# batmanlab/Mammo-CLIP

Measured on AMD Instinct MI355X. Metric: image-text pairs/s (whole node), EN-B5+BioClinicalBERT contrastive pre-training step, higher is better.
Workload: dtype bf16; 1 GPU; cfg4: efficientnet-b5 + BioClinicalBERT(BERT-base), 1024 pairs/GPU (2 views + 2 reports each), 1520x912 images, 256-token reports, breast_clip loss, AdamW; fwd+loss+bwd+optimizer; dropout/drop-connect on; global_batch=1024, parallelism=dp1 x 32 micro-batches, keep_graphs=7, recompute=0, keep_recompute=2, stat_tapes=True, streams=3

## Files before the change

### include/mammoclip_hip.h

```cpp
#ifndef MAMMOCLIP_HIP_H
#define MAMMOCLIP_HIP_H
#include <stdint.h>
#ifdef __cplusplus
extern "C" {
#endif

typedef uint16_t mc_bf16;

const char* mc_last_error(void);
int mc_version(void);
int mc_storage_is_f16(void);

typedef struct mc_gemm_args {
    const mc_bf16* A;
    const mc_bf16* B;
    void* C;
    long long M, K;
    int N;
    long long lda, ldb, ldc;
    int a_kmajor, b_kmajor;
    int c_f32, c_atomic;
    int splits;
    int batch, nb2;
    long long sA1, sA2, sB1, sB2, sC1, sC2;
// ... 28 lines not shown
int mc_quant_fp8_bf16(const mc_bf16* x, long long n, const float* amax_in, unsigned char* y, float* scale_out,
                      float* amax_next, void* stream);

typedef struct mc_gemm_rows_args {
    const mc_bf16* X;
    long long M;
    int K;
    long long ldx;
    const mc_bf16* W;
    int N;
    long long ldw;
    mc_bf16* C;
    long long ldc;
    const mc_bf16* R;
    long long ldr;
    const float* pro_scale;
    const float* pro_shift;
    const float* pro_gate;
    long long pro_rows_per_img;
    float* stat_partials;
    const float* bias;
    int epi_mode;
    const mc_bf16* epi_x;
    long long epi_ldx;
    long long epi_rows_per_img;
    const float* epi_scale;
    const float* epi_shift;
    const float* epi_mean;
    const float* epi_invstd;
    const float* epi_coef;
    const float* epi_mul;
    const float* epi_add;
    float epi_add_scale;
    float* epi_sums;
    float* epi_ws;
} mc_gemm_rows_args;
int mc_gemm_rows_supported(int n, int k);
long long mc_gemm_rows_epi_ws_floats(const mc_gemm_rows_args* args);
int mc_gemm_rows_epi_supported(long long M, int N, int K, long long rows_per_img, int epi_mode);
int mc_gemm_rows_blocks(const mc_gemm_rows_args* args);
int mc_gemm_rows_bf16(const mc_gemm_rows_args* args, void* stream);

typedef struct mc_wgrad_rows_args {
    const mc_bf16* dY;
    int N;
    long long lddy;
    const mc_bf16* X;
    int K;
    long long ldx;
    long long M;
    float* dW;
    float* ws;
    int accumulate;
    const float* pro_scale;
    const float* pro_shift;
    const float* pro_gate;
    long long pro_rows_per_img;
} mc_wgrad_rows_args;
int mc_wgrad_rows_supported(int n, int k);
int mc_wgrad_rows_blocks(long long m);
int mc_wgrad_rows_bf16(const mc_wgrad_rows_args* args, void* stream);
int mc_xbwd_rows_supported(int n, int k);
int mc_xbwd_rows_blocks(long long m);
int mc_xbwd_rows_bf16(const mc_wgrad_rows_args* args, const mc_bf16* wt, long long ldwt, mc_bf16* dx, long long lddx,
                      const mc_bf16* r, long long ldr, void* stream);

int mc_cast_f32_bf16(const float* src, mc_bf16* dst, long long n, void* stream);
int mc_cast_f32_bf16_lo(const float* src, mc_bf16* dst, long long n, void* stream);
int mc_cast_bf16_f32(const mc_bf16* src, float* dst, long long n, void* stream);
int mc_transpose_f32(const float* src, float* dst, int rows, int cols, void* stream);
int mc_cast_transpose_f32_bf16(const float* src, mc_bf16* dst, int rows, int cols, void* stream);
int mc_stem_weight_prep(const float* w, mc_bf16* out, int c0, void* stream);

int mc_stem_im2col(const float* x, long long sn, long long sc, long long sh, long long sw,
                   int n, int h, int w, int pad_l, int pad_t, int oh, int ow, mc_bf16* out, void* stream);
int mc_gate_weights_bf16(const mc_bf16* w, const float* gate, int n_img, int n, int k, mc_bf16* out, void* stream);

int mc_image_minmax_u8(const unsigned char* x, long long sn, long long elems_per_image, int n,
                       unsigned int* minmax, void* stream);
int mc_stem_im2col_u8(const unsigned char* x, long long sn, long long sc, long long sh, long long sw,
                      const unsigned int* minmax, float mean, float std, int n, int h, int w, int pad_l,
                      int pad_t, int oh, int ow, mc_bf16* out, void* stream);

typedef struct mc_dwconv_args {
    const mc_bf16* x;
    const mc_bf16* dy;
    void* out;
    const float* w_kkc;
    int n, h, w, c;
    int k, stride, pad_l, pad_t, oh, ow;
    const float* pro_scale;
    const float* pro_shift;
    float* stat_partials;
    const mc_bf16* epi_x;
    const float* epi_scale;
    const float* epi_shift;
    const float* epi_mean;
    const float* epi_invstd;
    float* dw_out;
    int stat_rows;
    const mc_bf16* xw;
    int cin;
} mc_dwconv_args;
int mc_dwconv_stat_rows(const mc_dwconv_args* args);
int mc_dwconv_bwd_data_stat_rows(const mc_dwconv_args* args);
int mc_dwconv_fwd(const mc_dwconv_args* args, void* stream);
int mc_dwconv_bwd_data(const mc_dwconv_args* args, void* stream);
int mc_dwconv_bwd_weight(const mc_dwconv_args* args, void* stream);
int mc_dwconv_bwd_data_xw_supported(const mc_dwconv_args* args);
int mc_dwconv_bwd_data_plan(const mc_dwconv_args* args, int* plan);
int mc_dwconv_bwd_data_xw_preferred(const mc_dwconv_args* args);
int mc_dwconv_set_lane_mode(int mode);
int mc_dwconv_lane_supported(const mc_dwconv_args* args);
int mc_dwconv_bwd_fused_supported(const mc_dwconv_args* args);
int mc_dwconv_bwd_fused_preferred(const mc_dwconv_args* args);
int mc_dwconv_bwd_fused_stat_rows(const mc_dwconv_args* args);
int mc_dwconv_bwd_fused(const mc_dwconv_args* args, void* stream);
int mc_mbconv_xdw_supported(const mc_dwconv_args* args);
int mc_mbconv_xdw_stat_rows(const mc_dwconv_args* args);
int mc_mbconv_xdw_fwd(const mc_dwconv_args* args, void* stream);

int mc_bn_finalize(const float* partials, int rows, int c, double count, const float* gamma,
                   const float* beta, float* running_mean, float* running_var, float momentum, float eps,
                   int update_running, float* mean, float* invstd, float* scale, float* shift, void* stream);
int mc_bn_eval_coeffs(const float* gamma, const float* beta, const float* running_mean,
                      const float* running_var, float eps, int c, float* scale, float* shift, void* stream);

typedef struct mc_bnact_args {
    const mc_bf16* x;
    long long n_img, hw;
    int c;
    const float* scale;
    const float* shift;
    int act;
    const float* rowscale;
    const mc_bf16* res;
    mc_bf16* out;
    float* pooled;
    const mc_bf16* g;
    const float* mul;
    const float* add;
    float add_scale;
    const float* mean;
    const float* invstd;
    float* partials;
    const float* coef;
    mc_bf16* dx;
    float* dgate;
    float* split_ws;
} mc_bnact_args;
int mc_bnact_rows(const mc_bnact_args* args);
int mc_bnact_img_splits(const mc_bnact_args* args);
int mc_bnact_apply(const mc_bnact_args* args, void* stream);
int mc_bnact_pool(const mc_bnact_args* args, void* stream);
int mc_bnact_bwd_reduce(const mc_bnact_args* args, void* stream);
int mc_bnact_bwd_apply(const mc_bnact_args* args, void* stream);
int mc_bnact_se_dgate(const mc_bnact_args* args, void* stream);
int mc_bnact_se_sums(const mc_bnact_args* args, void* stream);
int mc_bn_partials_from_se_sums(const float* sums, const float* gate, const float* dpooled, float add_scale,
                                long long n_img, int c, float* partials, void* stream);
int mc_bn_bwd_finalize(const float* partials, int rows, int c, double count, const float* gamma,
                       const float* mean, const float* invstd, float* dgamma, float* dbeta, float* coef,
                       void* stream);

int mc_bn_fold_prepare(const float* we, const float* coef, const float* xtx, const float* colsum_x, double rows, int n,
                       int k, mc_bf16* w1t, mc_bf16* wb, mc_bf16* sxx, void* stream);
// ... 135 lines not shown
```

### mammo_clip_amd/breastclip/model/modules/efficientnet_custom.py

```python
import math
from collections import namedtuple
from typing import List, Optional

import os

import torch
from torch import nn

from .... import ops

BN_MOMENTUM = 0.01
BN_EPS = 1e-3

VALID_MODELS = tuple(f"efficientnet-b{i}" for i in range(9)) + ("efficientnet-l2",)

_COEFFS = {
    "efficientnet-b0": (1.0, 1.0, 224, 0.2), "efficientnet-b1": (1.0, 1.1, 240, 0.2),
    "efficientnet-b2": (1.1, 1.2, 260, 0.3), "efficientnet-b3": (1.2, 1.4, 300, 0.3),
    "efficientnet-b4": (1.4, 1.8, 380, 0.4), "efficientnet-b5": (1.6, 2.2, 456, 0.4),
    "efficientnet-b6": (1.8, 2.6, 528, 0.5), "efficientnet-b7": (2.0, 3.1, 600, 0.5),
    "efficientnet-b8": (2.2, 3.6, 672, 0.5), "efficientnet-l2": (4.3, 5.3, 800, 0.5),
}
_STAGES = ((1, 3, 1, 1, 32, 16), (2, 3, 2, 6, 16, 24), (2, 5, 2, 6, 24, 40), (3, 3, 2, 6, 40, 80),
           (3, 5, 1, 6, 80, 112), (4, 5, 2, 6, 112, 192), (1, 3, 1, 6, 192, 320))
# ... 73 lines not shown
    _TAPE = tape


def _replaying():
    return _TAPE is not None and _TAPE.mode == "replay"


class _BNDefer:

    def __init__(self, enc):
        offs, tot = {}, 0
        for bn in enc._bn_layers:
            offs[id(bn)] = tot
            tot += bn.num_features
        self.offs, self.total = offs, tot
        self.flat = torch.zeros(2 * tot, dtype=torch.float32, device=enc._ones_b.device)
        self.used = []

    def scratch(self, bn):
        o, c = self.offs[id(bn)], bn.num_features
        self.used.append(bn)
        return self.flat[o:o + c], self.flat[self.total + o:self.total + o + c]

    @torch.no_grad()
    def apply(self):
        if not self.used:
            return
        if self.flat.is_cuda:
            self.flat.record_stream(torch.cuda.current_stream(self.flat.device))
        dst = [bn.running_mean for bn in self.used] + [bn.running_var for bn in self.used]
        src = [self.flat[self.offs[id(bn)]:self.offs[id(bn)] + bn.num_features] for bn in self.used] + \
              [self.flat[self.total + self.offs[id(bn)]:self.total + self.offs[id(bn)] + bn.num_features] for bn in self.used]
        torch._foreach_mul_(dst, 1.0 - BN_MOMENTUM)
        torch._foreach_add_(dst, src)
        self.used = []


_BN_DEFER = None


def _bn_stats(partials, count, bn: nn.BatchNorm2d, training: bool):
    if training:
        if _replaying():
            return _TAPE.get()
        if _BN_DEFER is not None and bn.track_update:
            rm, rv = _BN_DEFER.scratch(bn)
        else:
            rm, rv = bn.running_mean, bn.running_var
        st = ops.bn_finalize(partials, count, bn.weight, bn.bias, rm, rv, BN_MOMENTUM, BN_EPS, bn.track_update)
        if bn.track_update:
            if bn.defer_count is not None:
                bn.defer_count.append(bn.num_batches_tracked)
            else:
                bn.num_batches_tracked += 1
        if _TAPE is not None:
            _TAPE.put(st)
        return st
    return ops.bn_eval_coeffs(bn.weight, bn.bias, bn.running_mean, bn.running_var, BN_EPS)


def _conv_stats(fn, training, *a, stats=True, **kw):
    if not stats or (training and _replaying()):
        return fn(*a, **kw), None
    return fn(*a, stats=True, **kw)


LINK_STEM = os.environ.get("MC_LINK_STEM", "1") != "0"
FUSE_DW_BWD = os.environ.get("MC_FUSE_DW_BWD", "1") != "0"
FUSE_PROJ_DGRAD = os.environ.get("MC_FUSE_PROJ_DGRAD", "1") != "0"
BN_FOLD_MIN_BYTES = int(os.environ.get("MC_BN_FOLD_MIN_BYTES", 250_000_000))
BN_FOLD_S2_MIN_BYTES = int(os.environ.get("MC_BN_FOLD_S2_MIN_BYTES", 0))
XDW_MAX_CIN = int(os.environ.get("MC_XDW_MAX_CIN", 64))
MODE3_MAX_CEXP = int(os.environ.get("MC_MODE3_MAX_CEXP", 1 << 30))


class _StemFn(torch.autograd.Function):

    @staticmethod
    def forward(ctx, x, w, gamma, beta, mod, link=None):
        n, _, h, wd = x.shape
        l, r, t, b = mod.stem_pad
        _, oh, ow = mod.stem_geo(n, h, wd)
        c0 = w.shape[0]
        patches = ops.stem_im2col(x, l, t, oh, ow)
        wb = ops.stem_weight_prep(w)
        training = mod.training
        e, part = _conv_stats(ops.linear_fwd, training, patches, wb)
        st = _bn_stats(part, n * oh * ow, mod._bn0, training)
        ctx.mod, ctx.st, ctx.geo = mod, st, (n, h, wd, oh, ow, c0)
        ctx.raw = (x.mean, x.std) if isinstance(x, ops.RawImages) else None
        ctx.save_for_backward(x.data if ctx.raw else x, e)
        ctx.link = link
        if link is not None:
            link.st, link.part = st, None
            return e.detach()
        return ops.bnact_apply(e, n, oh * ow, c0, st.scale, st.shift, 1)

    @staticmethod
    def backward(ctx, dy):
        x, e = ctx.saved_tensors
        if ctx.raw:
            x = ops.RawImages(x, *ctx.raw)
        n, h, wd, oh, ow, c0 = ctx.geo
        mod = ctx.mod
        link = ctx.link
        if link is not None:
            de, dgamma, dbeta = ops.bnact_bwd(e, n, oh * ow, c0, ctx.st, mod._bn0.weight, 0, g=dy.contiguous(), partials=link.part)
            link.part = None
        else:
            de, dgamma, dbeta = ops.bnact_bwd(e, n, oh * ow, c0, ctx.st, mod._bn0.weight, 1, g=dy.contiguous())
        l, r, t, b = mod.stem_pad
        patches = ops.stem_im2col(x, l, t, oh, ow)
        dw = ops.linear_wgrad(de, patches)
        gw, gg, gb = ops.deliver_param_grads((mod._conv_stem.weight, mod._bn0.weight, mod._bn0.bias),
                                             (dw[:, :27].reshape(c0, 3, 3, 3), dgamma, dbeta))
        return (None, gw, gg, gb, None) + ((None,) if link is not None else ())


class _StemLink:
    __slots__ = ("st", "part")

    def __init__(self):
        self.st, self.part = None, None


def _expand_conv(pl, x, we, stats=True):
    if pl.fp8_expand:
        return ops.linear_fwd_fp8(x, we, stats=True)
    return _conv_stats(ops.linear_fwd, pl.training, x, we, stats=stats)


def _depthwise(blk, pl, x, e, we, wkkc, pro0, stats=True):
    if pl.xdw:
        return _conv_stats(ops.mbconv_xdw_fwd, pl.training, x, we, pro0, wkkc, *pl.dw, stats=stats)
    return _conv_stats(ops.dwconv_fwd, pl.training, e if blk.args.expand != 1 else x, wkkc, *pl.dw, stats=stats, pro=pro0)


def _project_conv(pl, d, act1, st1, gate, wp, stats=True):
    ohw = pl.oh * pl.ow
    if pl.fp8_project:
        wg = ops.gate_weights(wp, gate)
        return ops.linear_fwd_fp8(act1, wg, stats=True, batch_w=(pl.n, ohw))
    src, pro = (act1, (None, None, gate, ohw)) if pl.keep_act else (d, (st1.scale, st1.shift, gate, ohw))
    return _conv_stats(ops.linear_fwd, pl.training, src, wp, stats=stats, pro=pro)


class _MBConvFn(torch.autograd.Function):

    @staticmethod
    def forward(ctx, x, rowscale, blk, n, h, w, recording, link, *params):
        a = blk.args
        pl = blk.plan(n, h, w, recording)
        training, ohw = pl.training, pl.oh * pl.ow
        wkkc = blk.w_taps()
        e = we = st0 = gram = None
        if a.expand != 1:
            we = blk.w_expand()
            if pl.xdw:
                if training and _replaying():
                    part0, gram = None, _TAPE.get()
                elif training:
                    part0, gram = ops.bn_gram_partials(x, we, n * h * w)
                    if _TAPE is not None:
                        _TAPE.put(gram)
                else:
                    part0 = None
            else:
                e, part0 = _expand_conv(pl, x, we)
            st0 = _bn_stats(part0, n * h * w, blk._bn0, training)
            pro0 = (st0.scale, st0.shift)
        else:
            pro0 = (link.st.scale, link.st.shift) if link is not None else None
        d, part1 = _depthwise(blk, pl, x, e, we, wkkc, pro0)
        st1 = _bn_stats(part1, n * ohw, blk._bn1, training)
        if pl.keep_act:
            pooled, act1 = ops.bnact_pool(d, n, ohw, a.cexp, st1.scale, st1.shift, 1, keep_act=True)
        elif training and _replaying():
            pooled, act1 = _TAPE.get(), None
        else:
            pooled, act1 = ops.bnact_pool(d, n, ohw, a.cexp, st1.scale, st1.shift, 1), None
            if training and _TAPE is not None:
                _TAPE.put(pooled)
        if training and _replaying():
            gate = _TAPE.get()
        else:
            gate = ops.se_fwd(pooled, blk._se_reduce.weight.view(a.cse, a.cexp), blk._se_reduce.bias,
                              blk._se_expand.weight.view(a.cexp, a.cse), blk._se_expand.bias)
            if training and _TAPE is not None:
                _TAPE.put(gate)
        wp = blk.w_project()
        p, part2 = _project_conv(pl, d, act1, st1, gate, wp)
        st2 = _bn_stats(part2, n * ohw, blk._bn2, training)
        y = ops.bnact_apply(p, n, ohw, a.cout, st2.scale, st2.shift, 0,
                            rowscale=rowscale if a.skip else None, res=x if a.skip else None)
        ctx.blk, ctx.plan, ctx.saved = blk, pl, dict(
            x=x, e=e if pl.store_e else None, d=d if pl.store_d else None, act1=act1 if pl.store_d else None,
# ... 522 lines not shown
```

### mammo_clip_amd/lib.py

```python
import ctypes as C
import os

_HERE = os.path.dirname(os.path.abspath(__file__))
STORAGE = os.environ.get("MC_STORAGE", "bf16").lower()
if STORAGE not in ("bf16", "f16"):
    raise ValueError(f"MC_STORAGE must be 'bf16' or 'f16', got {STORAGE!r}")
LIB_PATH = os.path.join(_HERE, "lib", "libmammoclip_hip.so" if STORAGE == "bf16" else "libmammoclip_hip_f16.so")

P, LL, I, F, D, U, ULL = C.c_void_p, C.c_longlong, C.c_int, C.c_float, C.c_double, C.c_uint, C.c_ulonglong


class GemmArgs(C.Structure):
    _fields_ = [
        ("A", P), ("B", P), ("C", P),
        ("M", LL), ("K", LL), ("N", I),
        ("lda", LL), ("ldb", LL), ("ldc", LL),
        ("a_kmajor", I), ("b_kmajor", I),
        ("c_f32", I), ("c_atomic", I),
        ("splits", I),
        ("batch", I), ("nb2", I),
        ("sA1", LL), ("sA2", LL), ("sB1", LL), ("sB2", LL), ("sC1", LL), ("sC2", LL),
        ("bias", P), ("bias_stride1", LL),
        ("act", I),
        ("R", P), ("ldr", LL),
        ("alpha", F),
        ("pro_operand", I),
        ("pro_scale", P), ("pro_shift", P), ("pro_gate", P),
        ("pro_rows_per_img", LL), ("pro_nch", I),
        ("stat_partials", P),
        ("max_grid_m", I),
        ("splitk_ws", P),
        ("split_group_rows", LL), ("split_sub", I), ("split_scale", P),
        ("ab_fp8", I), ("alpha_dev", P),
    ]


class GemmRowsArgs(C.Structure):
    _fields_ = [
        ("X", P), ("M", LL), ("K", I), ("ldx", LL),
        ("W", P), ("N", I), ("ldw", LL),
        ("C", P), ("ldc", LL),
        ("R", P), ("ldr", LL),
        ("pro_scale", P), ("pro_shift", P), ("pro_gate", P), ("pro_rows_per_img", LL),
        ("stat_partials", P), ("bias", P),
        ("epi_mode", I), ("epi_x", P), ("epi_ldx", LL), ("epi_rows_per_img", LL),
        ("epi_scale", P), ("epi_shift", P), ("epi_mean", P), ("epi_invstd", P),
        ("epi_coef", P), ("epi_mul", P), ("epi_add", P), ("epi_add_scale", C.c_float),
        ("epi_sums", P), ("epi_ws", P),
    ]


class WgradRowsArgs(C.Structure):
    _fields_ = [
        ("dY", P), ("N", I), ("lddy", LL),
        ("X", P), ("K", I), ("ldx", LL),
        ("M", LL), ("dW", P), ("ws", P), ("accumulate", I),
        ("pro_scale", P), ("pro_shift", P), ("pro_gate", P), ("pro_rows_per_img", LL),
    ]


class DwconvArgs(C.Structure):
    _fields_ = [
        ("x", P), ("dy", P), ("out", P), ("w_kkc", P),
        ("n", I), ("h", I), ("w", I), ("c", I),
        ("k", I), ("stride", I), ("pad_l", I), ("pad_t", I), ("oh", I), ("ow", I),
        ("pro_scale", P), ("pro_shift", P), ("stat_partials", P),
        ("epi_x", P), ("epi_scale", P), ("epi_shift", P), ("epi_mean", P), ("epi_invstd", P),
        ("dw_out", P), ("stat_rows", I),
        ("xw", P), ("cin", I),
    ]


class BnactArgs(C.Structure):
    _fields_ = [
        ("x", P), ("n_img", LL), ("hw", LL), ("c", I),
        ("scale", P), ("shift", P), ("act", I),
        ("rowscale", P), ("res", P), ("out", P),
        ("pooled", P),
        ("g", P), ("mul", P), ("add", P), ("add_scale", F), ("mean", P), ("invstd", P),
        ("partials", P), ("coef", P), ("dx", P), ("dgate", P), ("split_ws", P),
    ]


class AdamwTensor(C.Structure):
    _fields_ = [("param", P), ("grad", P), ("exp_avg", P), ("exp_avg_sq", P), ("numel", LL), ("bf16_image", P)]


_SIGS = {
    "mc_version": ([], I),
    "mc_storage_is_f16": ([], I),
    "mc_adamw_step": ([C.POINTER(AdamwTensor), I, D, D, D, D, D, LL, P], I),
    "mc_grads_unscale": ([C.POINTER(AdamwTensor), I, F, P, P], I),
    "mc_grads_unscale_dev": ([C.POINTER(AdamwTensor), I, P, P, P], I),
    "mc_adamw_step_ls": ([C.POINTER(AdamwTensor), I, D, D, D, D, D, LL, P, P, P], I),
    "mc_loss_scale_update": ([P, P, D, D, I, I, P], I),
    "mc_grad_norm_partials": ([C.POINTER(AdamwTensor), I], LL),
    "mc_grad_norm": ([C.POINTER(AdamwTensor), I, P, LL, F, P, P], I),
    "mc_grads_unscale_norm_dev": ([C.POINTER(AdamwTensor), I, P, P, P, LL, F, P, P], I),
    "mc_grads_scale_dev": ([C.POINTER(AdamwTensor), I, P, P], I),
    "mc_adamw_step_clip": ([C.POINTER(AdamwTensor), I, D, D, D, D, D, LL, P, P, P, P], I),
    "mc_gemm_bf16": ([C.POINTER(GemmArgs), P], I),
    "mc_gemm_stat_rows": ([C.POINTER(GemmArgs)], I),
    "mc_gemm_tile_config": ([C.POINTER(GemmArgs)], I),
    "mc_gemm256_tn_eligible": ([C.POINTER(GemmArgs)], I),
    "mc_gemm256_tn_splits": ([LL, LL, LL, LL], I),
    "mc_amax_bf16": ([P, LL, P, P], I),
    "mc_quant_fp8_bf16": ([P, LL, P, P, P, P, P], I),
    "mc_gemm_rows_supported": ([I, I], I),
    "mc_gemm_rows_blocks": ([C.POINTER(GemmRowsArgs)], I),
    "mc_gemm_rows_epi_ws_floats": ([C.POINTER(GemmRowsArgs)], LL),
    "mc_gemm_rows_epi_supported": ([LL, I, I, LL, I], I),
    "mc_gemm_rows_bf16": ([C.POINTER(GemmRowsArgs), P], I),
    "mc_cast_transpose_f32_bf16": ([P, P, I, I, P], I),
    "mc_wgrad_rows_supported": ([I, I], I),
    "mc_wgrad_rows_blocks": ([LL], I),
    "mc_wgrad_rows_bf16": ([C.POINTER(WgradRowsArgs), P], I),
    "mc_xbwd_rows_supported": ([I, I], I),
    "mc_xbwd_rows_blocks": ([LL], I),
    "mc_xbwd_rows_bf16": ([C.POINTER(WgradRowsArgs), P, LL, P, LL, P, LL, P], I),
    "mc_cast_f32_bf16": ([P, P, LL, P], I),
    "mc_cast_bf16_f32": ([P, P, LL, P], I),
    "mc_cast_f32_bf16_lo": ([P, P, LL, P], I),
    "mc_transpose_f32": ([P, P, I, I, P], I),
    "mc_stem_weight_prep": ([P, P, I, P], I),
    "mc_stem_im2col": ([P, LL, LL, LL, LL, I, I, I, I, I, I, I, P, P], I),
    "mc_image_minmax_u8": ([P, LL, LL, I, P, P], I),
    "mc_gate_weights_bf16": ([P, P, I, I, I, P, P], I),
    "mc_stem_im2col_u8": ([P, LL, LL, LL, LL, P, F, F, I, I, I, I, I, I, I, P, P], I),
    "mc_dwconv_stat_rows": ([C.POINTER(DwconvArgs)], I),
    "mc_dwconv_bwd_data_stat_rows": ([C.POINTER(DwconvArgs)], I),
    "mc_dwconv_fwd": ([C.POINTER(DwconvArgs), P], I),
    "mc_dwconv_bwd_data": ([C.POINTER(DwconvArgs), P], I),
    "mc_dwconv_bwd_data_xw_supported": ([C.POINTER(DwconvArgs)], I),
    "mc_dwconv_bwd_data_plan": ([C.POINTER(DwconvArgs), C.POINTER(C.c_int)], I),
    "mc_dwconv_bwd_data_xw_preferred": ([C.POINTER(DwconvArgs)], I),
    "mc_dwconv_bwd_weight": ([C.POINTER(DwconvArgs), P], I),
    "mc_dwconv_set_lane_mode": ([I], I),
    "mc_dwconv_lane_supported": ([C.POINTER(DwconvArgs)], I),
    "mc_dwconv_bwd_fused_supported": ([C.POINTER(DwconvArgs)], I),
    "mc_dwconv_bwd_fused_preferred": ([C.POINTER(DwconvArgs)], I),
    "mc_dwconv_bwd_fused_stat_rows": ([C.POINTER(DwconvArgs)], I),
    "mc_dwconv_bwd_fused": ([C.POINTER(DwconvArgs), P], I),
    "mc_mbconv_xdw_supported": ([C.POINTER(DwconvArgs)], I),
    "mc_mbconv_xdw_stat_rows": ([C.POINTER(DwconvArgs)], I),
    "mc_mbconv_xdw_fwd": ([C.POINTER(DwconvArgs), P], I),
    "mc_bn_gram_partials": ([P, I, P, P, D, I, I, P, P], I),
    "mc_bn_finalize": ([P, I, I, D, P, P, P, P, F, F, I, P, P, P, P, P], I),
    "mc_bn_eval_coeffs": ([P, P, P, P, F, I, P, P, P], I),
    "mc_bnact_rows": ([C.POINTER(BnactArgs)], I),
    "mc_bnact_img_splits": ([C.POINTER(BnactArgs)], I),
    "mc_bnact_apply": ([C.POINTER(BnactArgs), P], I),
    "mc_bnact_pool": ([C.POINTER(BnactArgs), P], I),
    "mc_bnact_bwd_reduce": ([C.POINTER(BnactArgs), P], I),
    "mc_bnact_bwd_apply": ([C.POINTER(BnactArgs), P], I),
    "mc_bnact_se_dgate": ([C.POINTER(BnactArgs), P], I),
    "mc_bnact_se_sums": ([C.POINTER(BnactArgs), P], I),
    "mc_bn_partials_from_se_sums": ([P, P, P, F, LL, I, P, P], I),
    "mc_bn_bwd_finalize": ([P, I, I, D, P, P, P, P, P, P, P], I),
    "mc_colsum_rows": ([LL, I], I),
    "mc_colsum_bf16": ([P, LL, I, LL, P, P, I, P], I),
    "mc_se_fwd": ([P, P, P, P, P, I, I, I, P, P, P], I),
    "mc_se_bwd": ([P, P, P, P, P, P, P, I, I, I, P, P, P, P, P, P, P], I),
    "mc_dropout_f32": ([P, P, LL, F, ULL, U, P], I),
    "mc_bert_embed_fwd": ([P, P, P, P, P, P, P, F, I, I, I, F, ULL, U, P, P, P, P], I),
    "mc_bert_embed_bwd": ([P, P, P, P, P, P, P, P, P, I, I, I, F, ULL, U, P, P, P, P, P, P], I),
    "mc_add_ln_fwd": ([P, P, P, P, F, LL, I, F, ULL, U, P, P, P, P], I),
    "mc_add_ln_bwd": ([P, P, P, P, P, P, LL, I, F, ULL, U, P, P, P, P, P], I),
    "mc_softmax_fwd": ([P, LL, I, F, ULL, U, P, P, P], I),
    "mc_softmax_bwd": ([P, P, LL, I, F, ULL, U, F, P, P], I),
    "mc_bn_fold_prepare": ([P, P, P, P, D, I, I, P, P, P, P], I),
    "mc_bn_fold_cvec": ([P, P, P, P, P, D, I, I, P, P, P], I),
    "mc_bn_fold_wgrad": ([P, P, P, P, P, D, I, I, P, P], I),
    "mc_attn_supported": ([I, I], I),
    "mc_attn_fwd": ([P, P, I, I, I, F, F, ULL, U, P, P, P], I),
    "mc_attn_bwd": ([P, P, P, P, I, I, I, F, F, ULL, U, P, P], I),
    "mc_gelu_fwd": ([P, P, LL, P], I),
    "mc_gelu_bwd": ([P, P, P, LL, P], I),
    "mc_mask_bias": ([P, P, LL, P], I),
    "mc_eos_gather": ([P, P, I, I, I, P, P], I),
    "mc_eos_scatter": ([P, P, I, I, I, P, P], I),
    "mc_attn_varlen_supported": ([I, I], I),
    "mc_attn_varlen_fwd": ([P, P, P, I, I, I, LL, I, F, F, ULL, U, P, P, P], I),
    "mc_attn_varlen_bwd": ([P, P, P, P, P, I, I, I, LL, I, F, F, ULL, U, P, P], I),
    "mc_bert_embed_rows_fwd": ([P, P, P, P, P, P, P, P, P, F, LL, I, F, ULL, U, P, P, P, P], I),
    "mc_bert_embed_rows_bwd": ([P, P, P, P, P, P, P, P, P, P, I, I, I, I, F, ULL, U, P, P, P, P, P, P], I),
    "mc_add_ln_rows_fwd": ([P, P, P, P, P, F, LL, I, F, ULL, U, P, P, P, P], I),
    "mc_add_ln_rows_bwd": ([P, P, P, P, P, P, P, LL, I, F, ULL, U, P, P, P, P, P], I),
    "mc_rows_gather": ([P, P, I, I, P, P], I),
    "mc_rows_scatter": ([P, P, I, I, P, P], I),
    "mc_segment_mean_fwd": ([P, P, I, I, P, P], I),
    "mc_segment_mean_bwd": ([P, P, P, LL, I, I, P, P], I),
    "mc_unpack_rows": ([P, P, I, I, I, P, P], I),
    "mc_pack_rows": ([P, P, LL, I, P, P], I),
    "mc_sgemm": ([P, LL, LL, P, LL, LL, P, LL, I, I, I, F, F, P, P, P, P], I),
    "mc_sgemm_ws_floats": ([I, I, I], LL),
    "mc_scale_f32": ([P, P, F, P, LL, P], I),
    "mc_l2norm_fwd": ([P, I, I, P, P, P], I),
    "mc_l2norm_bwd": ([P, P, P, I, I, P, P], I),
    "mc_ce_fwd_bwd": ([P, I, I, P, I, F, F, P, P, P], I),
    "mc_sim_rank": ([P, P, P, P, I, I, I, P], I),
    "mc_sim_topk_ws_bytes": ([I, I, I], LL),
    "mc_sim_topk": ([P, P, P, P, I, I, I, I, P, P], I),
    "mc_sim_set_splits": ([I], I),
    "mc_sim_softmax": ([P, P, P, I, I, I, P], I),
    "mc_auroc_counts": ([P, P, P, I, P], I),
    "mc_augment_ws_bytes": ([I, I, I], LL),
    "mc_augment_u8": ([P, LL, LL, LL, I, P, I, P, I, I, I, P, P, LL, P], I),
    "mc_augment_set_stages": ([I], I),
}

EXPORTS = sorted(list(_SIGS.keys()) + ["mc_last_error"])
# ... 78 lines not shown
```

### mammo_clip_amd/ops.py

```python
import ctypes as C
import math
import os

import weakref

import torch

from . import lib as L

BF16 = torch.bfloat16 if L.STORAGE == "bf16" else torch.float16


def _p(t):
    return None if t is None else t.data_ptr()


_RAW_STREAM = getattr(torch._C, "_cuda_getCurrentRawStream", None)
_GET_DEV = getattr(torch._C, "_cuda_getDevice", None)


def _st():
    if _RAW_STREAM is None or _GET_DEV is None:
        return torch.cuda.current_stream().cuda_stream
    return _RAW_STREAM(_GET_DEV())
# ... 431 lines not shown

def cast_bf16_lo(src, out=None):
    def make():
        s_ = src.contiguous()
        dst = out if out is not None else empty(s_.shape, BF16, s_)
        L.call("mc_cast_f32_bf16_lo", _p(s_), _p(dst), s_.numel(), _st())
        return dst
    return make() if out is not None else _cached("clo", src, make)


def cast_f32(src):
    src = src.contiguous()
    dst = empty(src.shape, torch.float32, src)
    L.call("mc_cast_bf16_f32", _p(src), _p(dst), src.numel(), _st())
    return dst


def flipped_taps_f32(w_ck):
    def make():
        return transpose_f32(w_ck).flip(0).contiguous()
    return _cached("tfl", w_ck, make)


def transpose_f32(src, cache=False):
    def make():
        rows, cols = src.shape
        dst = empty((cols, rows), torch.float32, src)
        L.call("mc_transpose_f32", _p(src.contiguous()), _p(dst), rows, cols, _st())
        return dst
    return _cached("t", src, make) if cache else make()


def stem_weight_prep(w):
    c0 = w.shape[0]
    out = empty((c0, 32), BF16, w)
    L.call("mc_stem_weight_prep", _p(w.contiguous()), _p(out), c0, _st())
    return out


class RawImages:

    def __init__(self, data, mean, std):
        assert data.dtype == torch.uint8 and data.dim() == 4 and data.shape[1] == 3, "RawImages: uint8 [b,3,H,W]"
        self.data, self.mean, self.std = data, float(mean), float(std)

    def to(self, device, **kw):
        return RawImages(self.data.to(device, **kw), self.mean, self.std)

    shape = property(lambda self: self.data.shape)
    device = property(lambda self: self.data.device)
    is_cuda = property(lambda self: self.data.is_cuda)
    dtype = property(lambda self: self.data.dtype)


def image_minmax_u8(x):
    n = x.shape[0]
    per = x[0].numel()
    dense = sorted(zip(x.stride()[1:], x.shape[1:]), reverse=True)
    run = 1
    for st, sz in reversed(dense):
        assert sz == 1 or st == run, "RawImages: every image must be one dense block of bytes"
        run *= sz
    mm = torch.empty((2, n), dtype=torch.int32, device=x.device)
    L.call("mc_image_minmax_u8", _p(x), x.stride(0), per, n, _p(mm), _st())
    return mm


def stem_im2col(x, pad_l, pad_t, oh, ow):
    n, c, h, w = x.shape
    if isinstance(x, RawImages):
        d = x.data
        out = empty((n * oh * ow, 32), BF16, d)
        sn, sc, sh, sw = d.stride()
        L.call("mc_stem_im2col_u8", _p(d), sn, sc, sh, sw, _p(image_minmax_u8(d)), x.mean, x.std, n, h, w, pad_l, pad_t,
               oh, ow, _p(out), _st())
        return out
    assert c == 3 and x.dtype == torch.float32
    out = empty((n * oh * ow, 32), BF16, x)
    sn, sc, sh, sw = x.stride()
    L.call("mc_stem_im2col", _p(x), sn, sc, sh, sw, n, h, w, pad_l, pad_t, oh, ow, _p(out), _st())
    return out


def _dw_args(n, h, w, c, k, stride, pad_l, pad_t, oh, ow):
    a = L.DwconvArgs()
    a.n, a.h, a.w, a.c, a.k, a.stride, a.pad_l, a.pad_t, a.oh, a.ow = n, h, w, c, k, stride, pad_l, pad_t, oh, ow
    return a


def _dwconv_fwd_impl(x, w_kkc, n, h, w, c, k, stride, pad_l, pad_t, oh, ow, pro=None, stats=False, epi=None):
    a = _dw_args(n, h, w, c, k, stride, pad_l, pad_t, oh, ow)
    y = empty((n * oh * ow, c), BF16, x)
    a.x, a.out, a.w_kkc = _p(x), _p(y), _p(w_kkc)
    if pro is not None:
        a.pro_scale, a.pro_shift = _p(pro[0]), _p(pro[1])
    if epi is not None:
        e, st = epi
        assert stride == 1 and e.shape == y.shape
        a.epi_x, a.epi_scale, a.epi_shift, a.epi_mean, a.epi_invstd = _p(e), _p(st.scale), _p(st.shift), _p(st.mean), _p(st.invstd)
        stats = True
    part = None
    if stats:
        rows = L.load().mc_dwconv_stat_rows(C.byref(a))
        part = empty((rows, 2, c), torch.float32, x)
        a.stat_partials, a.stat_rows = _p(part), rows
    _note(2 * n * c * (h * w + oh * ow * (2 if epi is not None else 1)), 2 * n * c * oh * ow * k * k)
    L.call("mc_dwconv_fwd", C.byref(a), _st(), kind=f"k{k}s{stride}" + ("|dgrad_bn" if epi is not None else ""))
    return (y, part) if stats else y


def _dwconv_bwd_data_impl(dy, w_kkc, n, h, w, c, k, stride, pad_l, pad_t, oh, ow, w_kkc_flipped=None, epi=None, xw=None, dw=False):
    if stride == 1 and w_kkc_flipped is not None:
        assert xw is None and not dw
        return _dwconv_fwd_impl(dy, w_kkc_flipped, n, oh, ow, c, k, 1, k - 1 - pad_l, k - 1 - pad_t, h, w, epi=epi)
    assert epi is None or stride == 2
    if xw is not None:
        x, we = xw
        assert epi is not None and x.is_contiguous() and we.is_contiguous() and we.shape == (c, x.shape[1]) and x.shape[0] == n * h * w
        cin, st = x.shape[1], epi[1]
        a = _dw_args(n, h, w, c, k, stride, pad_l, pad_t, oh, ow)
        dz = empty((n * h * w, c), BF16, dy)
        a.dy, a.out, a.w_kkc = _p(dy), _p(dz), _p(w_kkc)
        a.epi_x, a.epi_scale, a.epi_shift, a.epi_mean, a.epi_invstd = _p(x), _p(st.scale), _p(st.shift), _p(st.mean), _p(st.invstd)
        a.xw, a.cin = _p(we), cin
        rows = L.load().mc_dwconv_bwd_data_stat_rows(C.byref(a))
        part = empty((rows, 2, c), torch.float32, dy)
        a.stat_partials, a.stat_rows = _p(part), rows
        dwdw = None
        if dw:
            dwdw = torch.zeros((k * k, c), dtype=torch.float32, device=dy.device)
            a.dw_out = _p(dwdw)
        _note(2 * n * (c * (oh * ow + h * w) + cin * h * w), (4 if dw else 2) * n * c * oh * ow * k * k + 2 * n * h * w * c * cin)
        L.call("mc_dwconv_bwd_data", C.byref(a), _st(), kind=f"k{k}s{stride}|dgrad_bn|x")
        return (dz, part, dwdw) if dw else (dz, part)
    assert not dw
    a = _dw_args(n, h, w, c, k, stride, pad_l, pad_t, oh, ow)
    dx = empty((n * h * w, c), BF16, dy)
    a.dy, a.out, a.w_kkc = _p(dy), _p(dx), _p(w_kkc)
    part = None
    if epi is not None:
        e, st = epi
        assert e.shape == dx.shape
        a.epi_x, a.epi_scale, a.epi_shift, a.epi_mean, a.epi_invstd = _p(e), _p(st.scale), _p(st.shift), _p(st.mean), _p(st.invstd)
        part = empty((L.load().mc_dwconv_bwd_data_stat_rows(C.byref(a)), 2, c), torch.float32, dy)
        a.stat_partials = _p(part)
    _note(2 * n * c * (h * w * (2 if epi is not None else 1) + oh * ow), 2 * n * c * oh * ow * k * k)
    L.call("mc_dwconv_bwd_data", C.byref(a), _st(), kind=f"k{k}s{stride}" + ("|dgrad_bn" if epi is not None else ""))
    return dx if epi is None else (dx, part)


def _dw_fused_args(dd, w_kkc_flipped, n, h, w, c, k, pad_l, pad_t, oh, ow, e, st, xw=None):
    a = _dw_args(n, oh, ow, c, k, 1, k - 1 - pad_l, k - 1 - pad_t, h, w)
    a.x, a.w_kkc = _p(dd), _p(w_kkc_flipped)
    a.epi_x, a.epi_scale, a.epi_shift, a.epi_mean, a.epi_invstd = _p(e), _p(st.scale), _p(st.shift), _p(st.mean), _p(st.invstd)
    if xw is not None:
        x, we = xw
        assert x.is_contiguous() and we.is_contiguous() and we.shape == (c, x.shape[1])
        a.epi_x, a.xw, a.cin = _p(x), _p(we), x.shape[1]
    return a


_FUSED_OK = {}


def dwconv_bwd_fused_ok(n, h, w, c, k, stride, pad_l, pad_t, oh, ow, force=False, cin=0):
    if stride != 1:
# ... 842 lines not shown
```

Before: 125.9 image-text pairs/s.

## Fuse stem im2col into conv GEMM for forward and weight-gradient kernels

Adds HIP kernels that gather the 3x3 stride-2 stem patches on the fly into LDS and run MFMA directly, instead of writing a full im2col patch matrix to HBM and then running a generic GEMM. The forward kernel also accumulates BN sum/sumsq partials. The wgrad kernel does per-block partial reductions plus a final reduce kernel. This removes a large patch-buffer write and read for the 1520x912 inputs. Forward fusion is only used in eval or graph replay unless MC_STEM_FUSED>=2, while the backward wgrad fusion is on by default.

```diff
diff --git a/include/mammoclip_hip.h b/include/mammoclip_hip.h
--- a/include/mammoclip_hip.h
+++ b/include/mammoclip_hip.h
@@ -134,6 +134,25 @@
                       const unsigned int* minmax, float mean, float std, int n, int h, int w, int pad_l,
                       int pad_t, int oh, int ow, mc_bf16* out, void* stream);
 
+typedef struct mc_stem_args {
+    const void* x;
+    long long sn, sc, sh, sw;
+    const unsigned int* minmax;
+    const mc_bf16* wb;
+    mc_bf16* e;
+    float* stat_partials;
+    float* dw;
+    float* ws;
+    float mean, std;
+    int src_u8;
+    int n, h, w, pad_l, pad_t, oh, ow;
+    int c0;
+} mc_stem_args;
+int mc_stem_fwd_blocks(const mc_stem_args* args);
+int mc_stem_fwd(const mc_stem_args* args, void* stream);
+int mc_stem_wgrad_blocks(const mc_stem_args* args);
+int mc_stem_wgrad(const mc_stem_args* args, void* stream);
+
 typedef struct mc_dwconv_args {
     const mc_bf16* x;
     const mc_bf16* dy;
diff --git a/mammo_clip_amd/breastclip/model/modules/efficientnet_custom.py b/mammo_clip_amd/breastclip/model/modules/efficientnet_custom.py
--- a/mammo_clip_amd/breastclip/model/modules/efficientnet_custom.py
+++ b/mammo_clip_amd/breastclip/model/modules/efficientnet_custom.py
@@ -179,10 +179,12 @@
         l, r, t, b = mod.stem_pad
         _, oh, ow = mod.stem_geo(n, h, wd)
         c0 = w.shape[0]
-        patches = ops.stem_im2col(x, l, t, oh, ow)
         wb = ops.stem_weight_prep(w)
         training = mod.training
-        e, part = _conv_stats(ops.linear_fwd, training, patches, wb)
+        if c0 <= 64 and (ops.STEM_FUSED >= 2 or (ops.STEM_FUSED and (not training or _replaying()))):
+            e, part = _conv_stats(ops.stem_fwd, training, x, wb, l, t, oh, ow, stats=training)
+        else:
+            e, part = _conv_stats(ops.linear_fwd, training, ops.stem_im2col(x, l, t, oh, ow), wb)
         st = _bn_stats(part, n * oh * ow, mod._bn0, training)
         ctx.mod, ctx.st, ctx.geo = mod, st, (n, h, wd, oh, ow, c0)
         ctx.raw = (x.mean, x.std) if isinstance(x, ops.RawImages) else None
@@ -207,8 +209,10 @@
         else:
             de, dgamma, dbeta = ops.bnact_bwd(e, n, oh * ow, c0, ctx.st, mod._bn0.weight, 1, g=dy.contiguous())
         l, r, t, b = mod.stem_pad
-        patches = ops.stem_im2col(x, l, t, oh, ow)
-        dw = ops.linear_wgrad(de, patches)
+        if ops.STEM_FUSED and c0 <= 64:
+            dw = ops.stem_wgrad(x, de, l, t, oh, ow)
+        else:
+            dw = ops.linear_wgrad(de, ops.stem_im2col(x, l, t, oh, ow))
         gw, gg, gb = ops.deliver_param_grads((mod._conv_stem.weight, mod._bn0.weight, mod._bn0.bias),
                                              (dw[:, :27].reshape(c0, 3, 3, 3), dgamma, dbeta))
         return (None, gw, gg, gb, None) + ((None,) if link is not None else ())
diff --git a/mammo_clip_amd/csrc/stem.hip b/mammo_clip_amd/csrc/stem.hip
--- /dev/null
+++ b/mammo_clip_amd/csrc/stem.hip
@@ -0,0 +1,382 @@
+#include "common_hip.h"
+#include "../../include/mammoclip_hip.h"
+
+namespace {
+
+constexpr int PROW = 80;
+
+template <typename SRC>
+struct Patch {
+    SRC r[27];
+    unsigned ok;
+    int img;
+};
+
+template <typename SRC>
+__device__ __forceinline__ void gather(const mc_stem_args& p, long long pix, long long M, Patch<SRC>& q) {
+    q.ok = 0u;
+    q.img = 0;
+#pragma unroll
+    for (int k = 0; k < 27; ++k) q.r[k] = (SRC)0;
+    if (pix >= M) return;
+    const unsigned ohw = (unsigned)p.oh * (unsigned)p.ow;
+    const unsigned img = (unsigned)pix / ohw, rem = (unsigned)pix - img * ohw;
+    const int oy = (int)(rem / (unsigned)p.ow), ox = (int)(rem - (unsigned)oy * (unsigned)p.ow);
+    q.img = (int)img;
+    const SRC* base = reinterpret_cast<const SRC*>(p.x) + (long long)img * p.sn;
+    const int ix0 = ox * 2 - p.pad_l, iy0 = oy * 2 - p.pad_t;
+    if (p.sc == 1 && p.sw == 3 && ix0 >= 0 && ix0 + 2 < p.w && iy0 >= 0 && iy0 + 2 < p.h) {
+        struct __attribute__((packed, aligned(sizeof(SRC)))) T3 { SRC a, b, c; };
+#pragma unroll
+        for (int kh = 0; kh < 3; ++kh) {
+            const SRC* rp = base + (long long)(iy0 + kh) * p.sh + (long long)ix0 * 3;
+#pragma unroll
+            for (int kw = 0; kw < 3; ++kw) {
+                const T3 t3 = *reinterpret_cast<const T3*>(rp + kw * 3);
+                q.r[0 * 9 + kh * 3 + kw] = t3.a;
+                q.r[1 * 9 + kh * 3 + kw] = t3.b;
+                q.r[2 * 9 + kh * 3 + kw] = t3.c;
+            }
+        }
+        q.ok = (1u << 27) - 1u;
+        return;
+    }
+#pragma unroll
+    for (int c = 0; c < 3; ++c)
+#pragma unroll
+        for (int kh = 0; kh < 3; ++kh) {
+            const int iy = iy0 + kh;
+#pragma unroll
+            for (int kw = 0; kw < 3; ++kw) {
+                const int ix = ix0 + kw;
+                if (iy >= 0 && iy < p.h && ix >= 0 && ix < p.w) {
+                    q.r[c * 9 + kh * 3 + kw] = base[c * p.sc + iy * p.sh + ix * p.sw];
+                    q.ok |= 1u << (c * 9 + kh * 3 + kw);
+                }
+            }
+        }
+}
+
+template <typename SRC>
+__device__ __forceinline__ void emit(const mc_stem_args& p, const Patch<SRC>& q, unsigned char* row) {
+    float v[32];
+#pragma unroll
+    for (int i = 27; i < 32; ++i) v[i] = 0.f;
+    if constexpr (sizeof(SRC) == 1) {
+        const float lo = (float)p.minmax[q.img];
+        const float range = (float)p.minmax[p.n + q.img] - lo;
+#pragma unroll
+        for (int k = 0; k < 27; ++k) {
+            float t = (float)q.r[k] - lo;
+            t = __fdiv_rn(t, range);
+            t = __fdiv_rn(__fsub_rn(t, p.mean), p.std);
+            v[k] = ((q.ok >> k) & 1u) ? t : 0.f;
+        }
+    } else {
+#pragma unroll
+        for (int k = 0; k < 27; ++k) v[k] = q.r[k];
+    }
+#pragma unroll
+    for (int j = 0; j < 4; ++j) *reinterpret_cast<uint4*>(row + j * 16) = pack8(v + j * 8);
+}
+
+template <typename SRC, int FN>
+__global__ __launch_bounds__(256, 2) void stem_fwd_k(const mc_stem_args p, const long long M, const long long ngroups, const long long gpb) {
+    constexpr int NP = FN * 16;
+    constexpr int CROW = (NP + 8) * 2;
+    constexpr int SC_BYTES = (4 * 16 * CROW > 4 * 64 * 16 * 4) ? 4 * 16 * CROW : 4 * 64 * 16 * 4;
+    __shared__ __attribute__((aligned(16))) unsigned char sW[FN * 1024];
+    __shared__ __attribute__((aligned(16))) unsigned char sP[4 * 64 * PROW];
+    __shared__ __attribute__((aligned(16))) unsigned char sC[SC_BYTES];
+    const int tid = threadIdx.x, lane = tid & 63, wave = tid >> 6;
+    const int N = p.c0;
+
+    for (int idx = tid; idx < FN * 64; idx += 256) {
+        const int l = idx & 63, f = idx >> 6;
+        const int n = f * 16 + (l & 15), k = (l >> 4) * 8;
+        uint4 v = make_uint4(0u, 0u, 0u, 0u);
+        if (n < N) v = *reinterpret_cast<const uint4*>(p.wb + n * 32 + k);
+        *reinterpret_cast<uint4*>(sW + (size_t)idx * 16) = v;
+    }
+    __syncthreads();
+    bf16x8_t wf[FN];
+#pragma unroll
+    for (int f = 0; f < FN; ++f) wf[f] = *reinterpret_cast<const bf16x8_t*>(sW + ((size_t)f * 64 + lane) * 16);
+
+    unsigned char* myP = sP + wave * 64 * PROW;
+    unsigned char* myC = sC + wave * 16 * CROW;
+    const int mrow = lane & 15, kg = lane >> 4;
+    const int cpr = N >> 3, slots = 64 / cpr;
+    const int c8 = lane % cpr, rs = lane / cpr;
+    const bool ep_active = rs < slots;
+    float ssum[8], ssq[8];
+#pragma unroll
+    for (int q = 0; q < 8; ++q) { ssum[q] = 0.f; ssq[q] = 0.f; }
+
+    const long long g_lo = (long long)blockIdx.x * gpb;
+    const long long g_hi = g_lo + gpb < ngroups ? g_lo + gpb : ngroups;
+    Patch<SRC> cur, nxt;
+    long long g = g_lo + wave;
+    if (g < g_hi) gather<SRC>(p, g * 64 + lane, M, cur);
+    for (; g < g_hi; g += 4) {
+        if (g + 4 < g_hi) gather<SRC>(p, (g + 4) * 64 + lane, M, nxt);
+        emit<SRC>(p, cur, myP + lane * PROW);
+        __builtin_amdgcn_wave_barrier();
+#pragma unroll
+        for (int rg = 0; rg < 4; ++rg) {
+            const long long mbase = g * 64 + rg * 16;
+            if (mbase >= M) break;
+            const bf16x8_t xf = *reinterpret_cast<const bf16x8_t*>(myP + (rg * 16 + mrow) * PROW + kg * 16);
+#pragma unroll
+            for (int f = 0; f < FN; ++f) {
+                const f32x4_t acc = MC_MFMA_16x16x32(wf[f], xf, ((f32x4_t){0.f, 0.f, 0.f, 0.f}), 0, 0, 0);
+                const uint2 pk = make_uint2(pack_bf2(acc[0], acc[1]), pack_bf2(acc[2], acc[3]));
+                *reinterpret_cast<uint2*>(myC + mrow * CROW + (f * 16 + kg * 4) * 2) = pk;
+            }
+            __builtin_amdgcn_wave_barrier();
+            if (ep_active) {
+                for (int row = rs; row < 16; row += slots) {
+                    const long long m = mbase + row;
+                    if (m < M) {
+                        const uint4 v = *reinterpret_cast<const uint4*>(myC + row * CROW + c8 * 16);
+                        if (p.stat_partials) {
+                            float a[8];
+                            unpack8(v, a);
+#pragma unroll
+                            for (int q = 0; q < 8; ++q) { ssum[q] += a[q]; ssq[q] += a[q] * a[q]; }
+                        }
+                        *reinterpret_cast<uint4*>(p.e + m * N + c8 * 8) = v;
+                    }
+                }
+            }
+            __builtin_amdgcn_wave_barrier();
+        }
+        cur = nxt;
+    }
+
+    if (p.stat_partials) {
+        __syncthreads();
+        float* red = reinterpret_cast<float*>(sC);
+#pragma unroll
+        for (int q = 0; q < 8; ++q) {
+            red[(wave * 64 + lane) * 16 + q] = ep_active ? ssum[q] : 0.f;
+            red[(wave * 64 + lane) * 16 + 8 + q] = ep_active ? ssq[q] : 0.f;
+        }
+        __syncthreads();
+        for (int c = tid; c < N; c += 256) {
+            float s = 0.f, s2 = 0.f;
+            for (int w = 0; w < 4; ++w)
+                for (int r = 0; r < slots; ++r) {
+                    const float* e = red + (w * 64 + r * cpr + (c >> 3)) * 16 + (c & 7);
+                    s += e[0]; s2 += e[8];
+                }
+            float* dst = p.stat_partials + (long long)blockIdx.x * 2 * N;
+            dst[c] = s;
+            dst[N + c] = s2;
+        }
+    }
+}
+
+typedef __attribute__((ext_vector_type(4))) short s4_t;
+typedef __attribute__((address_space(3))) s4_t lds_s4_t;
+__device__ __forceinline__ bf16x8_t tr_frag(const unsigned char* tile, int rs, int row0, int col0, int lane) {
+    const int g = lane >> 4, i = lane & 15;
+    const unsigned char* a = tile + (size_t)(row0 + g * 8 + (i >> 2)) * rs + (col0 + (i & 3) * 4) * 2;
+    s4_t lo = __builtin_amdgcn_ds_read_tr16_b64_v4i16((lds_s4_t*)(a));
+    s4_t hi = __builtin_amdgcn_ds_read_tr16_b64_v4i16((lds_s4_t*)(a + 4 * rs));
+    typedef __attribute__((ext_vector_type(8))) short s8_t;
+    s8_t v = {lo[0], lo[1], lo[2], lo[3], hi[0], hi[1], hi[2], hi[3]};
+    return __builtin_bit_cast(bf16x8_t, v);
+}
+
+template <typename SRC, int AF>
+__global__ __launch_bounds__(256, 2) void stem_wgrad_k(const mc_stem_args p, const long long M, const long long ngroups, const long long gpb) {
+    constexpr int NP = AF * 16;
+    constexpr int RSY = NP * 2 + 16;
+    constexpr int WTILE = 64 * (RSY + PROW);
+    __shared__ __attribute__((aligned(16))) unsigned char sT[4 * WTILE];
+    const int tid = threadIdx.x, lane = tid & 63, wave = tid >> 6;
+    const int N = p.c0, cpr = N >> 3;
+    unsigned char* myY = sT + wave * WTILE;
+    unsigned char* myX = myY + 64 * RSY;
+    for (int i = lane * 16; i < 64 * RSY; i += 64 * 16) *reinterpret_cast<uint4*>(myY + i) = make_uint4(0u, 0u, 0u, 0u);
+
+    f32x4_t acc[AF][2];
+#pragma unroll
+    for (int i = 0; i < AF; ++i) { acc[i][0] = (f32x4_t){0.f, 0.f, 0.f, 0.f}; acc[i][1] = (f32x4_t){0.f, 0.f, 0.f, 0.f}; }
+
+    int yrow[8], yoff[8];
+#pragma unroll
+    for (int i = 0; i < 8; ++i) {
+        const int c = lane + i * 64;
+        yrow[i] = c / cpr;
+        yoff[i] = yrow[i] * RSY + (c - yrow[i] * cpr) * 16;
+    }
+    auto load_de = [&](long long g, uint4 (&d)[8]) __attribute__((always_inline)) {
+#pragma unroll
+        for (int i = 0; i < 8; ++i) {
+            d[i] = make_uint4(0u, 0u, 0u, 0u);
+            if (i < cpr && g * 64 + yrow[i] < M)
+                d[i] = *reinterpret_cast<const uint4*>(p.e + g * 64 * N + (long long)(lane + i * 64) * 8);
+        }
+    };
+
+    const long long g_lo = (long long)blockIdx.x * gpb;
+    const long long g_hi = g_lo + gpb < ngroups ? g_lo + gpb : ngroups;
+    Patch<SRC> cur, nxt;
+    uint4 dcur[8], dnxt[8];
+    long long g = g_lo + wave;
+    if (g < g_hi) { gather<SRC>(p, g * 64 + lane, M, cur); load_de(g, dcur); }
+    for (; g < g_hi; g += 4) {
+        if (g + 4 < g_hi) { gather<SRC>(p, (g + 4) * 64 + lane, M, nxt); load_de(g + 4, dnxt); }
+        emit<SRC>(p, cur, myX + lane * PROW);
+#pragma unroll
+        for (int i = 0; i < 8; ++i)
+            if (i < cpr) *reinterpret_cast<uint4*>(myY + yoff[i]) = dcur[i];
+        __builtin_amdgcn_wave_barrier();
+#pragma unroll
+        for (int ks = 0; ks < 2; ++ks) {
+            bf16x8_t a[AF], b[2];
+#pragma unroll
+            for (int i = 0; i < AF; ++i) a[i] = tr_frag(myY, RSY, ks * 32, i * 16, lane);
+#pragma unroll
+            for (int j = 0; j < 2; ++j) b[j] = tr_frag(myX, PROW, ks * 32, j * 16, lane);
+#pragma unroll
+            for (int i = 0; i < AF; ++i)
+#pragma unroll
+                for (int j = 0; j < 2; ++j) acc[i][j] = MC_MFMA_16x16x32(a[i], b[j], acc[i][j], 0, 0, 0);
+        }
+        __builtin_amdgcn_wave_barrier();
+        cur = nxt;
+#pragma unroll
+        for (int i = 0; i < 8; ++i) dcur[i] = dnxt[i];
+    }
+
+    __syncthreads();
+    float* red = reinterpret_cast<float*>(sT);
+#pragma unroll
+    for (int i = 0; i < AF; ++i)
+#pragma unroll
+        for (int j = 0; j < 2; ++j) {
+            const int k = j * 16 + (lane & 15);
+#pragma unroll
+            for (int r = 0; r < 4; ++r) red[(wave * NP + i * 16 + (lane >> 4) * 4 + r) * 32 + k] = acc[i][j][r];
+        }
+    __syncthreads();
+    float* W = p.ws + (long long)blockIdx.x * N * 32;
+    for (int idx = tid; idx < N * 32; idx += 256) {
+        float s = red[idx];
+#pragma unroll
+        for (int w = 1; w < 4; ++w) s += red[w * NP * 32 + idx];
+        W[idx] = s;
+    }
+}
+
+__global__ __launch_bounds__(256) void stem_wgrad_reduce_k(const float* __restrict__ ws, int parts, int nk, float* __restrict__ out) {
+    __shared__ float sh[16][17];
+    const int el = threadIdx.x & 15, pl = threadIdx.x >> 4;
+    const int i = blockIdx.x * 16 + el;
+    float s = 0.f;
+    if (i < nk) {
+        int k = pl;
+        for (; k + 48 < parts; k += 64) {
+            const float a = ws[(long long)k * nk + i], b = ws[(long long)(k + 16) * nk + i];
+            const float c = ws[(long long)(k + 32) * nk + i], d = ws[(long long)(k + 48) * nk + i];
+            s += a; s += b; s += c; s += d;
+        }
+        for (; k < parts; k += 16) s += ws[(long long)k * nk + i];
+    }
+    sh[pl][el] = s;
+    __syncthreads();
+    if (pl != 0 || i >= nk) return;
+    s = 0.f;
+    for (int k = 0; k < 16; ++k) s += sh[k][el];
+    out[i] = s;
+}
+
+template <auto KERNEL> int stem_occupancy() {
+    static int occ = 0;
+    if (!occ) {
+        int nb = 0;
+        if (hipOccupancyMaxActiveBlocksPerMultiprocessor(&nb, reinterpret_cast<const void*>(KERNEL), 256, 0) != hipSuccess || nb < 1) nb = 2;
+        occ = nb > 4 ? 4 : nb;
+    }
+    return occ;
+}
+
+template <auto KERNEL> int launch_stem(const mc_stem_args& p, hipStream_t st, int* query) {
+    const long long M = (long long)p.n * p.oh * p.ow;
+    const long long ngroups = (M + 63) / 64;
+    long long b = (ngroups + 3) / 4;
+    const long long cap = 256LL * stem_occupancy<KERNEL>();
+    if (b > cap) b = cap;
+    const long long gpb = (ngroups + b - 1) / b;
+    b = (ngroups + gpb - 1) / gpb;
+    if (query) { *query = (int)b; return MC_OK; }
+    hipLaunchKernelGGL(KERNEL, dim3((unsigned)b), dim3(256), 0, st, p, M, ngroups, gpb);
+    MC_LAUNCH_CHECK();
+    return MC_OK;
+}
+
+template <typename SRC, bool WGRAD> int dispatch_stem(const mc_stem_args& p, hipStream_t st, int* query) {
+#define STEM_CASE(F_) case F_: return WGRAD ? launch_stem<stem_wgrad_k<SRC, F_>>(p, st, query) : launch_stem<stem_fwd_k<SRC, F_>>(p, st, query);
+    switch ((p.c0 + 15) / 16) {
+        STEM_CASE(1) STEM_CASE(2) STEM_CASE(3)
+        default: return WGRAD ? launch_stem<stem_wgrad_k<SRC, 4>>(p, st, query) : launch_stem<stem_fwd_k<SRC, 4>>(p, st, query);
+    }
+#undef STEM_CASE
+}
+template <bool WGRAD> int dispatch_src(const mc_stem_args& p, hipStream_t st, int* query) {
+    return p.src_u8 ? dispatch_stem<unsigned char, WGRAD>(p, st, query) : dispatch_stem<float, WGRAD>(p, st, query);
+}
+
+int check_stem(const mc_stem_args& p) {
+    MC_CHECK(p.n > 0 && p.h > 0 && p.w > 0 && p.oh > 0 && p.ow > 0, "stem: bad geometry");
+    MC_CHECK((long long)p.n * p.oh * p.ow < (1LL << 31), "stem: more than 2^31 output pixels");
+    MC_CHECK(p.c0 >= 8 && p.c0 <= 64 && p.c0 % 8 == 0, "stem: c0 must be a multiple of 8 up to 64");
+    return MC_OK;
+}
+int check_stem_src(const mc_stem_args& p) {
+    MC_CHECK(p.x && p.e && mc_aligned16(p.e), "stem: null image / e, or e not 16-byte aligned");
+    if (p.src_u8) MC_CHECK(p.minmax && p.std != 0.f, "stem (uint8 source): minmax / std");
+    else MC_CHECK(((uintptr_t)p.x & 3u) == 0, "stem: fp32 image must be 4-byte aligned");
+    return MC_OK;
+}
+
+}
+
+extern "C" int mc_stem_fwd_blocks(const mc_stem_args* a) {
+    int q = 0;
+    if (!a || check_stem(*a) != MC_OK) return 0;
+    return dispatch_src<false>(*a, nullptr, &q) == MC_OK ? q : 0;
+}
+
+extern "C" int mc_stem_fwd(const mc_stem_args* a, void* stream) {
+    MC_CHECK(a != nullptr, "stem_fwd: null args");
+    const mc_stem_args& p = *a;
+    if (check_stem(p) != MC_OK || check_stem_src(p) != MC_OK) return MC_ERR_ARG;
+    MC_CHECK(p.wb && mc_aligned16(p.wb), "stem_fwd: wb must be set and 16-byte aligned");
+    MC_CHECK(!p.stat_partials || mc_aligned16(p.stat_partials), "stem_fwd: stat_partials must be 16-byte aligned");
+    return dispatch_src<false>(p, (hipStream_t)stream, nullptr);
+}
+
+extern "C" int mc_stem_wgrad_blocks(const mc_stem_args* a) {
+    int q = 0;
+    if (!a || check_stem(*a) != MC_OK) return 0;
+    return dispatch_src<true>(*a, nullptr, &q) == MC_OK ? q : 0;
+}
+
+extern "C" int mc_stem_wgrad(const mc_stem_args* a, void* stream) {
+    MC_CHECK(a != nullptr, "stem_wgrad: null args");
+    const mc_stem_args& p = *a;
+    if (check_stem(p) != MC_OK || check_stem_src(p) != MC_OK) return MC_ERR_ARG;
+    MC_CHECK(p.dw && p.ws, "stem_wgrad: dw / ws");
+    int blocks = 0;
+    if (dispatch_src<true>(p, nullptr, &blocks) != MC_OK) return MC_ERR_ARG;
+    const int r = dispatch_src<true>(p, (hipStream_t)stream, nullptr);
+    if (r != MC_OK) return r;
+    const int nk = p.c0 * 32;
+    hipLaunchKernelGGL(stem_wgrad_reduce_k, dim3(mc_div_up(nk, 16)), dim3(256), 0, (hipStream_t)stream, p.ws, blocks, nk, p.dw);
+    MC_LAUNCH_CHECK();
+    return MC_OK;
+}
diff --git a/mammo_clip_amd/lib.py b/mammo_clip_amd/lib.py
--- a/mammo_clip_amd/lib.py
+++ b/mammo_clip_amd/lib.py
@@ -47,6 +47,17 @@
         ("epi_scale", P), ("epi_shift", P), ("epi_mean", P), ("epi_invstd", P),
         ("epi_coef", P), ("epi_mul", P), ("epi_add", P), ("epi_add_scale", C.c_float),
         ("epi_sums", P), ("epi_ws", P),
+    ]
+
+
+class StemArgs(C.Structure):
+    _fields_ = [
+        ("x", P), ("sn", LL), ("sc", LL), ("sh", LL), ("sw", LL),
+        ("minmax", P), ("wb", P), ("e", P), ("stat_partials", P),
+        ("dw", P), ("ws", P),
+        ("mean", F), ("std", F), ("src_u8", I),
+        ("n", I), ("h", I), ("w", I), ("pad_l", I), ("pad_t", I), ("oh", I), ("ow", I),
+        ("c0", I),
     ]
 
 
@@ -127,6 +138,10 @@
     "mc_image_minmax_u8": ([P, LL, LL, I, P, P], I),
     "mc_gate_weights_bf16": ([P, P, I, I, I, P, P], I),
     "mc_stem_im2col_u8": ([P, LL, LL, LL, LL, P, F, F, I, I, I, I, I, I, I, P, P], I),
+    "mc_stem_fwd_blocks": ([C.POINTER(StemArgs)], I),
+    "mc_stem_fwd": ([C.POINTER(StemArgs), P], I),
+    "mc_stem_wgrad_blocks": ([C.POINTER(StemArgs)], I),
+    "mc_stem_wgrad": ([C.POINTER(StemArgs), P], I),
     "mc_dwconv_stat_rows": ([C.POINTER(DwconvArgs)], I),
     "mc_dwconv_bwd_data_stat_rows": ([C.POINTER(DwconvArgs)], I),
     "mc_dwconv_fwd": ([C.POINTER(DwconvArgs), P], I),
diff --git a/mammo_clip_amd/ops.py b/mammo_clip_amd/ops.py
--- a/mammo_clip_amd/ops.py
+++ b/mammo_clip_amd/ops.py
@@ -537,6 +537,61 @@
     return out
 
 
+STEM_FUSED = int(os.environ.get("MC_STEM_FUSED", "1"))
+
+
+def _stem_args(x, pad_l, pad_t, oh, ow, c0):
+    n, c, h, w = x.shape
+    a = L.StemArgs()
+    if isinstance(x, RawImages):
+        d = x.data
+        a.keep = mm = image_minmax_u8(d)
+        a.src_u8, a.minmax, a.mean, a.std = 1, _p(mm), x.mean, x.std
+    else:
+        assert c == 3 and x.dtype == torch.float32
+        d = x
+    _chk_dev(d)
+    a.x = _p(d)
+    a.sn, a.sc, a.sh, a.sw = d.stride()
+    a.n, a.h, a.w, a.pad_l, a.pad_t, a.oh, a.ow, a.c0 = n, h, w, pad_l, pad_t, oh, ow, c0
+    return a, d
+
+
+def _stem_rows(entry, a):
+    rows = getattr(L.load(), entry)(C.byref(a))
+    if rows <= 0:
+        raise L.MammoClipHipError(f"{entry} refused the problem: " + L.load().mc_last_error().decode("utf-8", "replace"))
+    return rows
+
+
+def stem_fwd(x, wb, pad_l, pad_t, oh, ow, stats=False):
+    c0 = wb.shape[0]
+    a, d = _stem_args(x, pad_l, pad_t, oh, ow, c0)
+    assert wb.shape[1] == 32 and wb.is_contiguous() and wb.is_cuda
+    M = a.n * oh * ow
+    e = empty((M, c0), BF16, d)
+    a.wb, a.e = _p(wb), _p(e)
+    part = None
+    if stats:
+        part = empty((_stem_rows("mc_stem_fwd_blocks", a), 2, c0), torch.float32, d)
+        a.stat_partials = _p(part)
+    _note(d.numel() * d.element_size() + 2 * M * c0 + 2 * c0 * 32, 2 * M * c0 * 32)
+    L.call("mc_stem_fwd", C.byref(a), _st())
+    return (e, part) if stats else e
+
+
+def stem_wgrad(x, de, pad_l, pad_t, oh, ow):
+    M, c0 = de.shape
+    a, d = _stem_args(x, pad_l, pad_t, oh, ow, c0)
+    assert M == a.n * oh * ow and de.dtype == BF16 and de.is_contiguous() and de.is_cuda
+    dw = empty((c0, 32), torch.float32, d)
+    ws = empty((_stem_rows("mc_stem_wgrad_blocks", a), c0 * 32), torch.float32, d)
+    a.e, a.dw, a.ws = _p(de), _p(dw), _p(ws)
+    _note(d.numel() * d.element_size() + 2 * M * c0, 2 * M * c0 * 32)
+    L.call("mc_stem_wgrad", C.byref(a), _st())
+    return dw
+
+
 def _dw_args(n, h, w, c, k, stride, pad_l, pad_t, oh, ow):
     a = L.DwconvArgs()
     a.n, a.h, a.w, a.c, a.k, a.stride, a.pad_l, a.pad_t, a.oh, a.ow = n, h, w, c, k, stride, pad_l, pad_t, oh, ow
```

After: 126.3 image-text pairs/s, median of 6. About the same (+0.3%).
